# chlhnu/DOT-SOCP

Measured on AMD Instinct MI355X. Metric: ADMM iters/sec on NxNxT dot2d staggered grid at 1/2/4/8 MI355X, higher is better.
Workload: dtype f64

## Files before the change

### dot-socp_amd/capi.py

```python
import ctypes
import os

import numpy as np

_HERE = os.path.dirname(os.path.abspath(__file__))
LIB_PATH = os.path.join(_HERE, "lib", "libdotsocp.so")

i64 = ctypes.c_longlong
dbl = ctypes.c_double
vp = ctypes.c_void_p


class DotsocpError(RuntimeError):
    def __init__(self, code, msg):
        super().__init__(f"libdotsocp error {code}: {msg}")
        self.code = code


class Problem(ctypes.Structure):
    _fields_ = [("dim", ctypes.c_int), ("weighted", ctypes.c_int),
                ("ny", i64), ("nx", i64), ("nt", i64),
                ("D", dbl), ("E", dbl), ("cScale", dbl), ("dScale", dbl),
                ("normc", dbl), ("normd", dbl)]

# ... 16 lines not shown

METHOD_INPALM, METHOD_PALM, METHOD_ACCADMM = 0, 1, 2


F_PHI, F_Q, F_ALPHA, F_Z, F_BETA, F_C, F_WEIGHT = range(7)

SYMBOLS = {
    "dotsocp_last_error": (ctypes.c_char_p, []),
    "dotsocp_version": (ctypes.c_char_p, []),
    "dotsocp_device_count": (ctypes.c_int, []),
    "dotsocp_proj_soc": (ctypes.c_int, [vp, vp, i64, i64]),
    "dotsocp_bfd": (ctypes.c_int, [vp, vp, i64, i64, i64, dbl, dbl]),
    "dotsocp_bfd_conj": (ctypes.c_int, [vp, vp, i64, i64, i64, dbl]),
    "dotsocp_bfd1d": (ctypes.c_int, [vp, vp, i64, i64, dbl, dbl]),
    "dotsocp_bfd_conj1d": (ctypes.c_int, [vp, vp, i64, i64, dbl]),
    "dotsocp_oper_poisson": (ctypes.c_int, [vp, vp, i64, i64, i64, dbl]),
    "dotsocp_dctn": (ctypes.c_int, [vp, i64, i64, i64, ctypes.c_int]),
    "dotsocp_proj_soc_dev": (ctypes.c_int, [vp, vp, i64, i64, vp]),
    "dotsocp_bfd_dev": (ctypes.c_int, [vp, vp, i64, i64, i64, dbl, dbl, vp]),
    "dotsocp_bfd_conj_dev": (ctypes.c_int, [vp, vp, i64, i64, i64, dbl, vp]),
    "dotsocp_create": (vp, [ctypes.POINTER(Problem), ctypes.c_int, ctypes.c_int]),
    "dotsocp_create_multi": (vp, [ctypes.POINTER(Problem), ctypes.c_int, ctypes.c_int]),
    "dotsocp_destroy": (None, [vp]),
    "dotsocp_rccl_unique_id": (ctypes.c_int, [vp]),
    "dotsocp_attach_rccl": (ctypes.c_int, [vp, vp, ctypes.c_int, ctypes.c_int]),
    "dotsocp_slab_range": (ctypes.c_int, [i64, ctypes.c_int, ctypes.c_int, ctypes.POINTER(i64), ctypes.POINTER(i64)]),
    "dotsocp_field_len": (i64, [ctypes.POINTER(Problem), ctypes.c_int]),
    "dotsocp_dct_algorithm": (ctypes.c_int, [i64]),
    "dotsocp_dct_levels": (ctypes.c_int, [i64, ctypes.c_int]),
    "dotsocp_tsolve_tri_safe": (ctypes.c_int, [i64, i64, i64]),
    "dotsocp_cone_writes_beta": (ctypes.c_int, [i64, dbl, i64, ctypes.c_int, ctypes.c_int, ctypes.c_int, dbl, dbl]),
    "dotsocp_rescale_due": (ctypes.c_int, [i64, ctypes.c_int, dbl, dbl]),
    "dotsocp_qcone_form": (ctypes.c_int, [i64, dbl, i64, ctypes.c_int, ctypes.c_int, ctypes.c_int, ctypes.c_int, dbl, dbl]),
    "dotsocp_release_cache": (i64, []),
    "dotsocp_upload": (ctypes.c_int, [vp, ctypes.c_int, vp]),
    "dotsocp_upload_layers": (ctypes.c_int, [vp, ctypes.c_int, vp, i64, i64]),
    "dotsocp_download": (ctypes.c_int, [vp, ctypes.c_int, vp]),
    "dotsocp_begin": (ctypes.c_int, [vp, ctypes.POINTER(Opts)]),
    "dotsocp_begin_method": (ctypes.c_int, [vp, ctypes.POINTER(Opts), ctypes.c_int, ctypes.POINTER(AccOpts)]),
    "dotsocp_run": (ctypes.c_int, [vp, i64, ctypes.POINTER(i64)]),
    "dotsocp_recover_outputs": (ctypes.c_int, [vp, vp, vp, vp, vp, vp, vp, vp, vp]),
    "dotsocp_jump_next_level": (ctypes.c_int, [vp, vp]),
    "dotsocp_finish": (ctypes.c_int, [vp, ctypes.POINTER(Result)]),
    "dotsocp_get_history": (ctypes.c_int, [vp, vp, vp, vp, vp]),
    "dotsocp_set_profiling": (ctypes.c_int, [vp, ctypes.c_int]),
    "dotsocp_kernel_time": (ctypes.c_int, [vp, ctypes.c_char_p, ctypes.POINTER(dbl), ctypes.POINTER(i64)]),
    "dotsocp_canary_check": (ctypes.c_int, []),
    "dotsocp_poisson_phi": (ctypes.c_int, [vp]),
    "dotsocp_synchronize": (ctypes.c_int, [vp]),
    "dotsocp_weights_create": (vp, [ctypes.c_int, i64, i64, i64, ctypes.c_int]),
    "dotsocp_weights_destroy": (None, [vp]),
    "dotsocp_weights_len": (i64, [i64, i64, i64, ctypes.c_int, ctypes.c_int]),
    "dotsocp_weights_set": (ctypes.c_int, [vp, vp]),
    "dotsocp_weights_set_space": (ctypes.c_int, [vp, vp, vp]),
    "dotsocp_weights_restrict": (ctypes.c_int, [vp, ctypes.c_int]),
    "dotsocp_weights_log10_mean": (ctypes.c_int, [vp, ctypes.c_int, ctypes.POINTER(dbl)]),
    "dotsocp_weights_download": (ctypes.c_int, [vp, ctypes.c_int, vp]),
    "dotsocp_upload_weight_from": (ctypes.c_int, [vp, vp, ctypes.c_int]),
}

_lib = None


def _share_torchs_hip_runtime():
    import importlib.util
    import sys
# ... 68 lines not shown
```

### dot-socp_amd/csrc/capi.hip

```cpp
#include <cstring>
#include <new>

#include "comm.h"
#include "solver.h"
#include "weights.h"

using namespace dotsocp;

namespace dotsocp {
extern thread_local std::string g_last_error;
int dotsocp_slab_range_impl(i64 nt, int world, int rank, i64 *t0, i64 *t1);
}

struct dotsocp_ctx {
    Solver s;
};

struct dotsocp_weights {
    Weights w;
};

static int require_device() {
    int n = 0;
    if (hipGetDeviceCount(&n) != hipSuccess || n <= 0) {
// ... 243 lines not shown
    static_assert(sizeof(uid) == 128, "ncclUniqueId is expected to be 128 bytes");
    DS_NCCL(api.GetUniqueId(&uid));
    memcpy(id, &uid, sizeof uid);
    return 0;
}

int dotsocp_attach_rccl(dotsocp_ctx *ctx, const unsigned char id[128], int rank, int world) {
    if (!ctx) { set_error("ctx is NULL"); return DOTSOCP_EINVAL; }
    return ctx->s.attach_rccl(id, rank, world);
}

#define CTX_OR_FAIL()                                      \
    do {                                                   \
        if (!ctx) { set_error("ctx is NULL"); return DOTSOCP_EINVAL; } \
        (void)hipGetLastError();    \
    } while (0)

int dotsocp_dct_algorithm(dotsocp_i64 n) { return dct_choose_algorithm(n); }
int dotsocp_dct_levels(dotsocp_i64 n, int axis) { return dct_levels(n, axis); }
int dotsocp_tsolve_tri_safe(dotsocp_i64 ny, dotsocp_i64 nx, dotsocp_i64 nt) { return tsolve_tri_safe(ny, nx, nt) ? 1 : 0; }

int dotsocp_cone_writes_beta(dotsocp_i64 it, double last_sigma_it, dotsocp_i64 maxit, int check_step_by_step,
                             int last_of_run, int rescale, double maxFeas, double relGap) {
    return cone_writes_beta(it, last_sigma_it, maxit, check_step_by_step != 0, last_of_run != 0, rescale, maxFeas, relGap) ? 1 : 0;
}
int dotsocp_rescale_due(dotsocp_i64 it, int rescale, double maxFeas, double relGap) {
    return rescale_due(it, rescale, maxFeas, relGap) ? 1 : 0;
}
int dotsocp_qcone_form(dotsocp_i64 it, double last_sigma_it, dotsocp_i64 maxit, int check_step_by_step, int last_of_run,
                       int next_last_of_run, int rescale, double maxFeas, double relGap) {
    return qcone_form(it, last_sigma_it, maxit, check_step_by_step != 0, last_of_run != 0, next_last_of_run != 0, rescale,
                      maxFeas, relGap);
}

dotsocp_i64 dotsocp_field_len(const dotsocp_problem *p, int field) {
    if (!p || (p->dim != 1 && p->dim != 2) || p->nt < 2 || p->nx < 1 || (p->dim == 2 && p->ny < 1)) return -1;
    const i64 ny = p->dim == 1 ? p->nx : p->ny, nx = p->dim == 1 ? 1 : p->nx, nt = p->nt;
    const i64 Nphi = ny * nx * nt, Nz = ny * nx * (nt - 1);
    const i64 Nq = Nz + ny * (nx - 1) * nt + (ny - 1) * nx * nt;
    switch (field) {
        case DOTSOCP_F_PHI: case DOTSOCP_F_C: return Nphi;
        case DOTSOCP_F_Q: case DOTSOCP_F_ALPHA: case DOTSOCP_F_WEIGHT: return Nq;
        case DOTSOCP_F_Z: case DOTSOCP_F_BETA: return Nz * (p->dim == 1 ? 6 : 10);
        default: return -1;
    }
}

int dotsocp_upload(dotsocp_ctx *ctx, int field, const double *host) { CTX_OR_FAIL(); return ctx->s.upload(field, host); }
dotsocp_i64 dotsocp_release_cache(void) { return (dotsocp_i64)device_cache_release(); }

int dotsocp_upload_layers(dotsocp_ctx *ctx, int field, const double *host, dotsocp_i64 t0, dotsocp_i64 n) {
    CTX_OR_FAIL();
    return ctx->s.upload_layers(field, host, t0, n);
}
int dotsocp_download(dotsocp_ctx *ctx, int field, double *host) { CTX_OR_FAIL(); return ctx->s.download(field, host); }
int dotsocp_begin(dotsocp_ctx *ctx, const dotsocp_opts *opts) { CTX_OR_FAIL(); return ctx->s.begin(opts); }
int dotsocp_begin_method(dotsocp_ctx *ctx, const dotsocp_opts *opts, int method, const dotsocp_acc_opts *acc) {
    CTX_OR_FAIL();
    return ctx->s.begin_method(opts, method, acc);
}
int dotsocp_recover_outputs(dotsocp_ctx *ctx, const double *rho0, const double *rho1, double *rho, double *Ex,
                            double *Ey, double *q0, double *bx, double *by) {
    CTX_OR_FAIL();
    if (ctx->s.prob.dim == 1)
        return ctx->s.recover_outputs(rho0, rho1, rho, nullptr, Ex, q0, nullptr, bx);
    return ctx->s.recover_outputs(rho0, rho1, rho, Ex, Ey, q0, bx, by);
// ... 102 lines not shown
```

### dot-socp_amd/csrc/kernels.h

```cpp
#pragma once
#include "common.h"
#include "defer.h"

namespace dotsocp {

struct LoopCoef {
    double s;
    double sf;
    double dF;
    double at, ax, ay;
    double tau;
    double c1, c2;
    double dinv1, dinv2;
};

enum {
    S_Q2 = 0, S_Z2, S_APHI2, S_ALPHA2, S_BETA2, S_FBBETA2, S_PRIM1, S_PRIM2, S_DUAL1, S_DUAL2,
    S_COMPLEM, S_DOTCOMP, S_RHO2, S_RHOFQ2, S_MRHOB, S_M2, S_RHOB2, S_QALPHA, S_CPHI, S_PHI2,
    S_COUNT
};

struct KktCoef {
    double sigma;
    double kappa;
// ... 84 lines not shown

int launch_prolong_phi(const Grid &gf, const Grid &gc, const double *phic, double *phif, double sc_in, double sc_out,
                       hipStream_t st, i64 tc0 = 0);
int launch_prolong_beta(const Grid &gf, const Grid &gc, const double *betac, double *betaf, double *neg, double sc_in0,
                        double sc_in1, double sc_out, hipStream_t st, i64 tc0 = 0, i64 Nzc = -1);
int launch_scale_div(double *x, const double *w, i64 n, double sc, hipStream_t st);
int launch_fill(double *x, i64 n, double v, hipStream_t st);
int launch_outputs(const Grid &g, const double *q, const double *alpha, const double *weight, const double *rho0,
                   const double *rho1, const double *a_prev, double sig, double cD, double dD, int which, double *out,
                   hipStream_t st);
int launch_out_tail(const Grid &g, const double *alpha, const double *weight, double sig, double cD, double *out,
                    hipStream_t st);

struct QStepExtra {
    ScaleOps aops;
    double *partials, *resid;
    double kappa, dsD;
    double *u0_tail;
    int c_ends;
};
int launch_qstep_rhs(const Grid &g, const LoopCoef &c, const FusedGeom &fg, const double *phi, const double *q2,
                     const double *sx, const double *sy, const double *weight, const double *tail_bx,
                     const double *tail_by, const double *cvec, double *q_out, const double *alpha_in, double *alpha_out,
                     double *rhs, hipStream_t st, i64 z0 = 0, i64 zcount = -1, i64 zstride = 1,
                     const QStepExtra *ex = nullptr);
i64 qstep_rhs_blocks(const Grid &g, const FusedGeom &fg);
struct QConeArgs {
    const double *phi, *q2v, *sx, *sy, *cvec, *alpha_in, *gamma_in;
    double *alpha_out, *rhs, *q_out, *beta_out, *q2_out, *sx_out, *sy_out;
    i64 TC;
    int ap_on;
    double ap_mul, ap_div;
    int c_ends;
};
int launch_qcone(const Grid &g, const LoopCoef &c, const FusedGeom &fg, QConeArgs a, bool gout, hipStream_t st);
i64 qcone_chunk_len(const Grid &g);
i64 qstep_rhs_chunks(const Grid &g, const FusedGeom &fg, i64 *TC = nullptr);
int launch_qstep_rhs_acc(int var, const Grid &g, const LoopCoef &c, const FusedGeom &fg, const double *phi,
                         const double *q2, const double *sx, const double *sy, const double *weight, const double *cvec,
                         double *q_raw, const double *alpha_in, double *alpha_out, double *rhs, double *q_state,
                         const double *q_anchor, const double *alpha_anchor, const AccCoef &k, hipStream_t st,
                         const double *tail_bx = nullptr, const double *tail_by = nullptr, double *u0_tail = nullptr);
int launch_qstep_palm_first(const Grid &g, const LoopCoef &c, const FusedGeom &fg, const double *phi, const double *q2,
                            const double *sx, const double *sy, const double *cvec, double *q_out, const double *alpha,
                            double *rhs, hipStream_t st, const double *tail_bx = nullptr, const double *tail_by = nullptr,
                            const double *qk = nullptr);

int launch_qstep_fused(const Grid &g, const LoopCoef &c, const FusedGeom &fg, const double *phi,
                       const double *q2, const double *sx, const double *sy, const double *weight,
                       const double *tail_bx, const double *tail_by, double *q_out, double *alpha,
                       hipStream_t st);
int launch_rhs_sigma_fix(const Grid &g, double *rhs, const double *r, double *cvec, double factor, hipStream_t st,
                         bool c_ends = false);
int launch_c_interior_test(const Grid &g, const double *cvec, int *flag, hipStream_t st);
int launch_rhs_fixup(const Grid &g, const LoopCoef &c, const double *u0_prev, double *rhs, hipStream_t st);
int launch_grad(const Grid &g, const LoopCoef &c, const double *phi, double *out, hipStream_t st);
int launch_tail_finalize(const Grid &g, const LoopCoef &c, const FusedGeom &fg, const double *q2, const double *sx,
                         const double *sy, double *tail_bx, double *tail_by, hipStream_t st);
int launch_kkt_tail(const Grid &g, const double *alpha, const double *beta, const double *weight, double *a0,
                    double *a0w, double *bt_bx, double *bt_by, hipStream_t st);
int launch_rhs(const Grid &g, const LoopCoef &c, const double *q, const double *alpha, const double *cvec,
               const double *weight, const double *u0_prev, double *rhs, hipStream_t st, bool c_ends = false);
int launch_qstep(const Grid &g, const LoopCoef &c, const double *phi, const double *z, const double *beta,
                 const double *weight, const double *tail_bx, const double *tail_by, double *q,
                 double *alpha, hipStream_t st);
int launch_u0_tail(const Grid &g, const double *q, const double *alpha, const double *weight, double *out,
                   hipStream_t st);
int launch_scale(double *x, i64 n, double mul, double div, hipStream_t st);
// ... 79 lines not shown
```

### dot-socp_amd/csrc/qstep_march.hip

```cpp
#include "device_utils.h"
#include "gather_tile.h"
#include "kernels.h"
#include "qstep_tile.h"

#include <cstdlib>

namespace dotsocp {


struct QRhsArgs {
    const double *phi, *q2v, *sx, *sy, *weight, *tail_bx, *tail_by, *cvec, *alpha_in;
    double *q_out, *alpha_out, *rhs;
    double *u0_tail;
    i64 TC, z0, zstride;
    double *q_state;
    const double *q_anchor, *alpha_anchor;
    double c1, c2, om_rho, rho;
    APend ap;
    int xcd;
    const double *qk;
    double *partials, *resid;
    double kappa, dsD;
    int c_ends;
};
// ... 234 lines not shown
    if (z0 < 0 || zcount <= 0 || zstride < 1 || z0 + (zcount - 1) * zstride >= chunks) return 0;
    a.TC = TC;
    a.z0 = z0;
    a.zstride = zstride;
    a.xcd = 1;
    dim3 grid((unsigned)fg.nyblk, (unsigned)fg.nxblk, (unsigned)zcount);
    dim3 blk(TILE_Y, TILE_X);
    const char *qe = getenv("DOTSOCP_QTX");
    const int qtx_env = qe ? atoi(qe) : 0;
    const int qtx = qtx_env ? qtx_env : ((fg.nyblk * fg.nxblk * zcount >= 8192 && !a.weight) ? 2 * TILE_X : TILE_X);
    if (var == 0 && !a.partials && qtx == 2 * TILE_X) {
        dim3 grid2((unsigned)fg.nyblk, (unsigned)((g.nx + 2 * TILE_X - 1) / (2 * TILE_X)), (unsigned)zcount);
        dim3 blk2(TILE_Y, 2 * TILE_X);
        if (a.weight) DS_KLAUNCH((k_qstep_rhs<true, 0, false, 2 * TILE_X>), grid2, blk2, 0, st, g, c, fg, a);
        else DS_KLAUNCH((k_qstep_rhs<false, 0, false, 2 * TILE_X>), grid2, blk2, 0, st, g, c, fg, a);
        DS_HIP(hipGetLastError());
        return 0;
    }
#define QRHS_LAUNCH(W, V) DS_KLAUNCH((k_qstep_rhs<W, V>), grid, blk, 0, st, g, c, fg, a)
    if (var == 0 && a.partials) {
        if (a.weight) DS_KLAUNCH((k_qstep_rhs<true, 0, true>), grid, blk, 0, st, g, c, fg, a);
        else DS_KLAUNCH((k_qstep_rhs<false, 0, true>), grid, blk, 0, st, g, c, fg, a);
    } else if (a.weight) {
        if (var == 0) QRHS_LAUNCH(true, 0); else if (var == 1) QRHS_LAUNCH(true, 1); else QRHS_LAUNCH(true, 2);
    } else {
        if (var == 0) QRHS_LAUNCH(false, 0); else if (var == 1) QRHS_LAUNCH(false, 1);
        else if (var == 2) QRHS_LAUNCH(false, 2); else QRHS_LAUNCH(false, 3);
    }
#undef QRHS_LAUNCH
    DS_HIP(hipGetLastError());
    return 0;
}

template <bool NT, bool GOUT>
__global__ void __launch_bounds__(TILE_Y *TILE_X, 3) k_qcone(Grid g, LoopCoef c, FusedGeom fg, QConeArgs a) {
    constexpr int XB = TILE_X;
    __shared__ double2 xch[2][XB][TILE_Y];
    __shared__ double ph[2][XB + 2][TILE_Y + 2];
    __shared__ double2 gch[2][XB][64];
    const APend ap{a.ap_on, a.ap_mul, a.ap_div};
    const BlockId blk = block_id(true);
    const QTile<XB> t = q_tile<XB>(g, fg, blk);
    const int lane = t.lane, xl = t.xl;
    const i64 y = t.y, x = t.x;
    const bool inb = t.inb;
    const i64 t0 = (i64)blk.z * a.TC;
    const i64 t1 = (t0 + a.TC < g.ntl) ? t0 + a.TC : g.ntl;
    const i64 tstart = (t0 >= 2) ? t0 - 2 : 0;
    const i64 tstop = (t1 == g.ntl) ? t1 + 1 : t1;
    const i64 nxblk = gridDim.y, nyblk = gridDim.x;
    const QSrc src{a.phi, a.q2v, a.sx, a.sy, nullptr, nullptr, nullptr, a.cvec, a.alpha_in, nullptr, a.c_ends};
    double p0 = 0.0;
    if (inb) {
        const i64 node0 = y + g.py * (x + g.nx * tstart);
        p0 = a.phi[node0];
        store_phi_layer<XB>(ph[0], t, p0, load_phi_halo(g, t, a.phi, node0));
    }
    double u0prev = 0.0;
    double q0c = 0.0;
    EdgeQuad eprev{0.0, 0.0, 0.0, 0.0};
    GatherCarry gc;
    int par = 0;
    __syncthreads();
    for (i64 tl = tstart; tl < tstop; ++tl) {
        const bool own = tl >= t0;
        const bool hasC = (tl > tstart) && (tl - 1 < g.ncl);
        const i64 ci = t.yc + g.py * (t.xc + g.nx * (hasC ? tl - 1 : 0));
        double b[10];
        if (hasC) {
#pragma unroll
            for (int j = 0; j < 10; ++j) b[j] = ld_stream<NT>(a.gamma_in + j * g.Nc + ci);
        }
        EdgeQuad ecur{0.0, 0.0, 0.0, 0.0};
        double q0n = 0.0;
        if (tl < g.ntl) {
            const QLayerIn in = q_layer_load<false, XB>(g, c, fg, t, src, ph[par], tl, false, false);
            const QLayerOut o = q_layer_calc<false, 0, XB>(c, t, in, ap, p0, false, false);
            q0n = o.q0n;
            if (own) {
                if (in.hasCell) {
                    a.alpha_out[in.node] = o.a0n;
                    if (!GOUT) a.q_out[in.node] = o.q0n;
                }
                if (t.hasBx) {
                    a.alpha_out[in.eX] = o.aXn;
                    if (!GOUT) a.q_out[in.eX] = o.qXn;
                }
                if (t.hasBy) {
                    a.alpha_out[in.eY] = o.aYn;
                    if (!GOUT) a.q_out[in.eY] = o.qYn;
                }
            }
            xch[par][xl][lane] = make_double2(o.ubx, o.qXn);
            store_phi_layer<XB>(ph[par ^ 1], t, in.pTl, in.h);
            __syncthreads();
            const double uby_s = __shfl_up(o.uby, 1, 64);
            const double qY_s = __shfl_up(o.qYn, 1, 64);
            if (inb) {
                const double2 r = from_left(t, xch[par], make_double2(o.ubx_l, o.qL),
                                            make_double2(0.0, 0.0));
                const double uby_m = from_below(t, uby_s, o.uby_b), qY_m = from_below(t, qY_s, o.qB);
                if (own) a.rhs[in.node] = adjoint_sum(g, c, t, tl, u0prev, o.u0, r.x, o.ubx, uby_m, o.uby) + in.cv;
                ecur.xm = (x >= 1) ? c.sf * r.y : 0.0;
                ecur.xp = (x <= g.nx - 2) ? c.sf * o.qXn : 0.0;
                ecur.ym = (y >= 1) ? c.sf * qY_m : 0.0;
                ecur.yp = (y <= g.ny - 2) ? c.sf * o.qYn : 0.0;
            }
            u0prev = o.u0;
            p0 = o.pT;
            par ^= 1;
        }
        if (tl > tstart) {
            double w[10];
            if (hasC) {
                double v[10];
                build_z2(v, q0c, eprev, ecur, c.s, c.dF);
#pragma unroll
                for (int j = 0; j < 10; ++j) b[j] = mult_finish(b[j], v[j], c.tau);
                if (!GOUT && own && inb) {
#pragma unroll
                    for (int j = 0; j < 10; ++j) st_stream<NT>(a.beta_out + j * g.Nc + ci, b[j]);
                }
#pragma unroll
                for (int j = 0; j < 10; ++j) v[j] = v[j] - b[j];
                proj_row<10>(v);
                if (GOUT && own && inb) {
#pragma unroll
                    for (int j = 0; j < 10; ++j) st_stream<NT>(a.beta_out + j * g.Nc + ci, mult_carry(b[j], v[j], c.tau));
                }
#pragma unroll
                for (int j = 0; j < 10; ++j) w[j] = v[j] + b[j];
                if (own && inb) a.q2_out[ci] = c.s * (w[9] - w[0]);
            } else {
#pragma unroll
                for (int j = 0; j < 10; ++j) w[j] = 0.0;
            }
            gather_emit<XB>(g, c.sf, gch, gc, w, tl - 1, own && inb, x, y, xl, lane, nxblk, nyblk, blk.y, blk.x, a.q2_out,
                            a.sx_out, a.sy_out);
        }
        eprev = ecur;
        q0c = q0n;
    }
}

i64 qcone_chunk_len(const Grid &g) {
    i64 TC = g.ntl;
    if (const char *e = getenv("DOTSOCP_QCONE_TC")) {
        const i64 n = atoll(e);
        if (n >= 1) TC = n;
    }
    return TC < g.ntl ? TC : g.ntl;
}

int launch_qcone(const Grid &g, const LoopCoef &c, const FusedGeom &fg, QConeArgs a, bool gout, hipStream_t st) {
    if (fg.XB != TILE_X || !(g.first && g.last) || g.ncl < 1) { set_error("internal: k_qcone on a grid it does not serve"); return DOTSOCP_ESTATE; }
    a.TC = qcone_chunk_len(g);
    const i64 chunks = (g.ntl + a.TC - 1) / a.TC;
    dim3 grid((unsigned)fg.nyblk, (unsigned)fg.nxblk, (unsigned)chunks);
    dim3 blk(TILE_Y, TILE_X);
    const bool nt = stream_nt_enabled();
    if (gout) {
        if (nt) DS_KLAUNCH((k_qcone<true, true>), grid, blk, 0, st, g, c, fg, a);
        else DS_KLAUNCH((k_qcone<false, true>), grid, blk, 0, st, g, c, fg, a);
    } else {
        if (nt) DS_KLAUNCH((k_qcone<true, false>), grid, blk, 0, st, g, c, fg, a);
        else DS_KLAUNCH((k_qcone<false, false>), grid, blk, 0, st, g, c, fg, a);
    }
    DS_HIP(hipGetLastError());
    return 0;
}

int launch_qstep_palm_first(const Grid &g, const LoopCoef &c, const FusedGeom &fg, const double *phi, const double *q2,
                            const double *sx, const double *sy, const double *cvec, double *q_out, const double *alpha,
                            double *rhs, hipStream_t st, const double *tail_bx, const double *tail_by, const double *qk) {
    QRhsArgs a{};
    a.phi = phi; a.q2v = q2; a.sx = sx; a.sy = sy; a.cvec = cvec; a.tail_bx = tail_bx; a.tail_by = tail_by;
    a.alpha_in = alpha; a.q_out = q_out; a.rhs = rhs; a.qk = qk;
    return launch_qstep_rhs_var(3, g, c, fg, a, st);
}

}
```

### dot-socp_amd/csrc/solver.h

```cpp
#pragma once
#include <chrono>
#include <functional>
#include <memory>
#include <string>
#include <vector>

#include "hostmem.h"
#include "kernels.h"

namespace dotsocp {

int guarded_malloc(void **p, size_t bytes);
void guarded_free(void *p);
long long device_cache_release();
int canary_check(std::string *report);
bool canary_enabled();
bool stream_stress_enabled();
void stream_stress(hipStream_t st);

template <class T>
inline int dmalloc(T **p, i64 n) {
    *p = nullptr;
    if (n <= 0) n = 1;
    return guarded_malloc((void **)p, sizeof(T) * (size_t)n);
// ... 47 lines not shown
    double *u0_prev = nullptr, *tail_bx = nullptr, *tail_by = nullptr;
    double *a0_prev = nullptr, *a0w_prev = nullptr, *btail_bx = nullptr, *btail_by = nullptr;
    double *send_plane = nullptr, *send_plane2 = nullptr, *send_bx = nullptr, *send_by = nullptr;
    KktWork kw{};
    double *q_old = nullptr, *q2 = nullptr, *beta2 = nullptr, *sx = nullptr, *sy = nullptr;
    double *q3 = nullptr, *p2 = nullptr, *sxp = nullptr, *syp = nullptr;
    double *send_pbx = nullptr, *send_pby = nullptr, *ptail_bx = nullptr, *ptail_by = nullptr;
    double *alpha2 = nullptr;
    double *sx2 = nullptr, *sy2 = nullptr;
    double *tri_send = nullptr, *tri_recv = nullptr, *tri_bsend = nullptr, *tri_brecv = nullptr, *tri_zero = nullptr;
    double *carry = nullptr;
    FusedGeom fg{};
    double *phi_p = nullptr, *alpha_p = nullptr, *z_p = nullptr;
    double *phi_a = nullptr, *q_a = nullptr, *alpha_a = nullptr, *z_a = nullptr, *beta_a = nullptr;
};

#define FOR_SLABS(s) for (auto &s : slabs) if (int rc_use__ = use(s)) return rc_use__; else

int dotsocp_slab_range_impl(i64 nt, int world, int rank, i64 *t0, i64 *t1);
void pencil_range(i64 plane, int world, int j, i64 *l0, i64 *l1);

bool if_adjust_sigma(double iter, double last_iter);

enum Phase { PH_RHS = 0, PH_POISSON, PH_PROJ, PH_QSTEP, PH_BETA, PH_KKT, PH_FUSED_A, PH_FUSED_B, PH_MATERIALISE,
             PH_COMM, PH_INTERP, PH_ACC_CONE, PH_ACC_GATHER, PH_QSTEP0, PH_TRANSPOSE, PH_CONE_CARRY, PH_QCONE, PH_COUNT };

bool rescale_due(i64 it, int rescale, double maxFeas, double relGap);
bool cone_writes_beta(i64 it, double lastSigmaIt, i64 maxit, bool checkStepByStep, bool last_of_run, int rescale,
                      double maxFeas, double relGap);

enum { QCONE_NONE = 0, QCONE_STEADY = 1, QCONE_EXIT = 2 };
int qcone_form(i64 it, double lastSigmaIt, i64 maxit, bool checkStepByStep, bool last_of_run, bool next_last_of_run,
               int rescale, double maxFeas, double relGap);

struct Solver {
    dotsocp_problem prob{};
    int device = 0;
    i64 ny = 0, nx = 0, nt = 0;
    hipStream_t stream = nullptr;
    hipStream_t stream_z = nullptr;
    bool multi_device = false;
    int ndev_visible = 1;
    std::vector<DevRes *> devres;
    int cur_dev = -1;
    std::vector<Slab> slabs;
    std::unique_ptr<DeferCtx> defer;
    int world = 1;
    int rank = 0;
    void *nccl = nullptr;
    double *h_sums = nullptr;
    double *d_red = nullptr;
    bool fused = true;
    bool overlap = false;
    bool tri_tsolve = true;
    bool peer_ok = true;
    bool cross_device = false;
    ~Solver();
    int init(const dotsocp_problem *p, int device, int nslabs, bool multi_dev = false);
    int attach_rccl(const unsigned char *id, int rank, int world);
    int use(const Slab &s);
    int use_dev(int d);
    int sync_all();
    DevRes *res_for(int dev);
    i64 column_pad() const;
    i64 row_pitch() const;
    int alloc_slabs(int first, int count);
// ... 52 lines not shown
    int upload_weight_from(const double *src, int src_dev, i64 src_ny, i64 src_nx, i64 src_nt);
    bool c_ends_on = true;
    int detect_c_ends();
    int recover_outputs(const double *rho0, const double *rho1, double *rho, double *Ex, double *Ey, double *q0,
                        double *bx, double *by);
    int jump_from(Solver &coarse);

    bool begun = false, finished = false, stopped = false;
    dotsocp_opts opts{};
    bool checkPrimDualFeas = true;
    double time_limit = 3600.0;
    double sigma = 1.0, sigmaScale = 1.0;
    double cScale = 1.0, dScale = 1.0, D = 1.0, E = 1.0;
    double norm_c = 0.0, norm_d = 0.0;
    double h = 1.0;
    int rescale = 0, use_feasOrg = 0;
    double maxFeas = 0.0, relGap = 0.0, tol_feasOrg = 0.0;
    double lastSigmaIt = 0.0;
    i64 it = 0;
    LoopCoef lc{};
    std::vector<double> hist_kkt, hist_time, hist_iter, hist_gap;
    std::chrono::steady_clock::time_point t_begin;
    double elapsed_prev = 0.0;
    double elapsed_agreed = 0.0;
    bool deferred = false;
    bool z_valid = true;
    bool z_prev_ok = false;
    bool rhs_valid = false;
    bool cone_carry = true;
    bool beta_gamma = false;
    bool cone_gout = false;
    bool last_of_run = false;
    int qcone = -1;
    bool q_valid = true;
    bool early_pass = false;
    bool early_gout = false;
    bool next_last_of_run = false;
    int need_q(const char *who) const;
    int qcone_decide() const;
    bool time_limit_passed() const;
    i64 timeout_at = -1;
    bool timeout_pending = false;
    int need_beta_form(const char *who) const;
    ScaleOps bops{0, 1.0, 1.0, 1.0, 1.0};
    ScaleOps zp_ops{0, 1.0, 1.0, 1.0, 1.0};
    int push_beta_op(double mul, double div);
    int flush_beta();
    ScaleOps aops{0, 1.0, 1.0, 1.0, 1.0};
    int flush_alpha();
    int sigma_scale_folded(double factor);
    FusedArgs pending_step_args(const Slab &s) const;
    double last_S[S_COUNT] = {0};
    double last_S_sigma = 1.0;
    i64 last_S_it = -1;
    bool norm_cache = true;
    bool kkt_fold = true;
    KktCoef kkt_coef() const;
    int clear_partials(Slab &s);
    int begin(const dotsocp_opts *o);
    int begin_method(const dotsocp_opts *o, int method, const dotsocp_acc_opts *acc);
    int run(i64 n_iters, i64 *done);
    int finish(dotsocp_result *res);
    int step(bool *brk);
    int rescale_block();
    int poisson_all(const PhiHooks *hooks = nullptr);
    int poisson_phi();
// ... 48 lines not shown
```

### dot-socp_amd/csrc/solver.hip

```cpp
#include "solver.h"

#include <algorithm>
#include <cmath>
#include <cstring>

#include "comm.h"

namespace dotsocp {

void Solver::update_coef() {
    lc.s = E / D;
    lc.sf = edge_factor(lc.s);
    lc.dF = E / dScale;
    const double ht = 1.0 / (double)(nt - 1);
    lc.at = D * (1.0 / ht);
    lc.ax = (nx > 1) ? D * (1.0 / (1.0 / (double)(nx - 1))) : 0.0;
    lc.ay = (ny > 1) ? D * (1.0 / (1.0 / (double)(ny - 1))) : 0.0;
    lc.tau = opts.tau;
    const double tmp = (E / D) * (E / D);
    if (prob.weighted) { lc.c1 = 2.0 * tmp; lc.c2 = tmp; }
    else { lc.c1 = 1.0 + 2.0 * tmp; lc.c2 = 1.0 + tmp; }
    lc.dinv1 = 1.0 / lc.c1;
    lc.dinv2 = 1.0 / lc.c2;
}
// ... 94 lines not shown
    if (m == DOTSOCP_METHOD_INPALM) return begin(o);
    DS_ARG(m == DOTSOCP_METHOD_ACCADMM || m == DOTSOCP_METHOD_PALM, "unknown method");
    DS_ARG(prob.dim == 2, "the reference has PALM and acc-ADMM loops for 2-D problems only");
    DS_ARG(!(m == DOTSOCP_METHOD_PALM && prob.weighted), "the reference has no weighted PALM loop");
    method = m;
    int rc = begin(o);
    if (rc != 0) { method = DOTSOCP_METHOD_INPALM; return rc; }
    return (m == DOTSOCP_METHOD_PALM) ? palm_begin() : acc_begin(acc);
}

int Solver::begin(const dotsocp_opts *o) {
    DS_ARG(o != nullptr, "opts is NULL");
    DS_ARG(o->maxit >= 0, "opts.maxit < 0");
    DS_ARG(o->sigma > 0, "opts.sigma must be positive");
    if (begun) { set_error("begin() called twice"); return DOTSOCP_ESTATE; }
    cur_dev = -1;
    DS_CHECK(use_dev(device));
    DS_CHECK(ensure_alloc());
    if (method == DOTSOCP_METHOD_ACCADMM) {
        DS_CHECK(acc_alloc());
        fused = false;
    }
    opts = *o;
    cone_carry = true;
    if (const char *e = getenv("DOTSOCP_CONE_CARRY")) cone_carry = (atoi(e) != 0);
    c_ends_on = true;
    if (const char *e = getenv("DOTSOCP_C_ENDS")) c_ends_on = (atoi(e) != 0);
    if (c_ends_on) DS_CHECK(detect_c_ends());
    timeout_at = -1;
    if (const char *e = getenv("DOTSOCP_TEST_TIMEOUT_AT")) timeout_at = atoll(e);
    qcone = -1;
    if (const char *e = getenv("DOTSOCP_QCONE")) qcone = atoi(e);
    if (qcone < -1 || qcone > 2) qcone = -1;
    q_valid = true;
    early_pass = false;
    early_gout = false;
    next_last_of_run = false;
    beta_gamma = false;
    cone_gout = false;
    last_of_run = false;
    timeout_pending = false;
    checkPrimDualFeas = (o->checkPrimDualFeas < 0) ? !prob.weighted : (o->checkPrimDualFeas != 0);
    time_limit = (o->time_limit > 0) ? o->time_limit : 3600.0;
    sigma = o->sigma;
    lastSigmaIt = -INFINITY;
    cScale = prob.cScale; dScale = prob.dScale; D = prob.D; E = prob.E;
    use_feasOrg = 0;
    tol_feasOrg = 5 * o->tol;
    rescale = o->scaling ? 1 : 0;
    maxFeas = INFINITY; relGap = INFINITY;
    h = 1.0 / ((double)nx * (double)ny * (double)nt);
    norm_c = prob.normc; norm_d = prob.normd;
    update_coef();
    DS_CHECK(scale_state(1.0, sigma, 1.0, true));
    DS_CHECK(exchange_q_halo(false));
    sigmaScale = 1.0;
    it = 0;
    stopped = false;
    deferred = false;
    z_valid = true;
    z_prev_ok = false;
    rhs_valid = false;
    last_S_it = -1;
    hist_kkt.clear(); hist_time.clear(); hist_iter.clear(); hist_gap.clear();
    for (int i = 0; i < PH_COUNT; ++i) { phase_ms[i] = 0; phase_launches[i] = 0; }
    if (canary_enabled() && getenv("DOTSOCP_CANARY_SELFTEST")) {
// ... 142 lines not shown
        }
        const int mode = deferred ? 1 : 0;
        if (s.carry && C > 1) {
            for (i64 z = z0; z < z0 + zc; ++z) {
                a.carry_in = (z > 0) ? s.carry : nullptr;
                a.carry_out = (z + 1 < C) ? s.carry : nullptr;
                DS_CHECK(launch_cone_fused(mode, s.g, lc, s.fg, a, s.st, z, 1, flavour));
            }
        } else {
            DS_CHECK(launch_cone_fused(mode, s.g, lc, s.fg, a, s.st, z0, zc, flavour));
        }
        if (deferred && part != 1) std::swap(s.beta, s.beta2);
    }
    prof_end(ph);
    if (part == 1) return 0;
    if (deferred) {
        bops.clear();
        beta_gamma = gout;
    }
    return 0;
}

KktCoef Solver::kkt_coef() const {
    KktCoef k;
    k.sigma = sigma;
    k.kappa = sigma * cScale * D;
    k.dsD = dScale / D;
    k.dsE = dScale / E;
    return k;
}

int Solver::phase_q(int part, bool kkt, int early) {
    if (!fused) DS_CHECK(flush_alpha());
    if (early != QCONE_NONE && (part != 0 || kkt || multi() || !fused || !deferred || !beta_gamma || !bops.empty())) {
        set_error("internal: early cone pass in a state it does not serve");
        return DOTSOCP_ESTATE;
    }
    const bool egout = (early == QCONE_STEADY);
    const int ph = (early != QCONE_NONE) ? PH_QCONE : PH_QSTEP;
    prof_begin(ph);
    FOR_SLABS(s) {
        hipStream_t st = s.st;
        if (early != QCONE_NONE && qcone != 2) {
            if (!s.sx2) {
                DS_CHECK(s.zalloc(&s.sx2, s.fg.sx_len));
                DS_CHECK(s.zalloc(&s.sy2, s.fg.sy_len));
            }
            QConeArgs a{};
            a.phi = s.phi; a.q2v = s.q2; a.sx = s.sx; a.sy = s.sy; a.cvec = s.c; a.alpha_in = s.alpha; a.gamma_in = s.beta;
            a.alpha_out = s.alpha2; a.rhs = s.w0; a.q_out = s.q_old; a.beta_out = s.beta2;
            a.q2_out = s.q; a.sx_out = s.sx2; a.sy_out = s.sy2;
            a.ap_on = aops.n; a.ap_mul = aops.mul; a.ap_div = aops.div;
            a.c_ends = (c_ends_on && s.c_ends) ? 1 : 0;
            DS_CHECK(launch_qcone(s.g, lc, s.fg, a, egout, st));
            std::swap(s.alpha, s.alpha2);
            std::swap(s.q, s.q_old);
            std::swap(s.q2, s.q_old);
            std::swap(s.sx, s.sx2);
            std::swap(s.sy, s.sy2);
            std::swap(s.beta, s.beta2);
        } else if (!fused) {
            DS_CHECK(launch_qstep(s.g, lc, s.phi, s.z, s.beta, s.weight, s.tail_bx, s.tail_by, s.q, s.alpha, s.st));
        } else {
            const i64 C = qstep_rhs_chunks(s.g, s.fg);
            i64 z0 = 0, zc = C, zs = 1;
            if (part == 1) { zc = C - 1; }
            else if (part == 2) { z0 = C - 1; zc = 1; }
            QStepExtra ex{};
            ex.aops = aops;
            ex.c_ends = (c_ends_on && s.c_ends) ? 1 : 0;
            if (multi() && !s.g.last && part != 1) ex.u0_tail = s.send_plane;
            if (kkt) {
                const KktCoef k = kkt_coef();
                ex.partials = kkt_qstep_partials(s.g, s.kw);
                ex.resid = s.w1;
                ex.kappa = k.kappa; ex.dsD = k.dsD;
            }
            DS_CHECK(launch_qstep_rhs(s.g, lc, s.fg, s.phi, s.q2, s.sx, s.sy, s.weight, s.tail_bx, s.tail_by, s.c,
                                      s.q_old, s.alpha, s.alpha2, s.w0, st, z0, zc, zs, &ex));
            if (part != 1) std::swap(s.alpha, s.alpha2);
            if (part != 1) std::swap(s.q, s.q_old);
            if (early != QCONE_NONE) {
                FusedArgs a{};
                a.q = s.q; a.q2 = s.q2; a.sx = s.sx; a.sy = s.sy;
                a.beta_in = s.beta; a.beta_out = s.beta2;
                a.bops = bops;
                DS_CHECK(launch_cone_fused(1, s.g, lc, s.fg, a, s.st, 0, s.fg.chunks, CONE_GIN | (egout ? CONE_GOUT : 0)));
                std::swap(s.beta, s.beta2);
            }
        }
    }
    prof_end(ph);
    if (part == 1) return 0;
    q_valid = true;
    if (early != QCONE_NONE) {
        q_valid = !egout || qcone == 2;
        beta_gamma = egout;
        z_valid = false;
        z_prev_ok = false;
        early_pass = true;
        early_gout = egout;
    }
    u0_made = multi() && fused;
    if (fused) aops.clear();
    rhs_valid = fused;
    if (multi() && fused && comm_z && cone_split_enabled()) halo_pending = true;
    else DS_CHECK(exchange_q_halo(true));
    return 0;
}

int Solver::phase_mult() {
    if (fused) {
        deferred = true;
        return 0;
    }
    prof_begin(PH_BETA);
    FOR_SLABS(s) DS_CHECK(launch_beta_update(s.g, lc, s.q, s.z, s.beta, s.st));
    prof_end(PH_BETA);
    return 0;
}

int Solver::materialise() {
    if (!fused || !deferred) return 0;
    DS_CHECK(need_beta_form("materialise"));
    DS_CHECK(need_q("materialise"));
    DS_CHECK(ensure_halo());
    prof_begin(PH_MATERIALISE);
    FOR_SLABS(s) {
        FusedArgs a = pending_step_args(s);
        a.beta_out = s.beta;
        a.z_out = s.z;
        DS_CHECK(launch_cone_fused(2, s.g, lc, s.fg, a, s.st));
    }
    prof_end(PH_MATERIALISE);
// ... 172 lines not shown
    DS_CHECK(scale_state(dScale2, cScale2 * cScale2, dScale2, true));
    if (method == DOTSOCP_METHOD_PALM) {
        FOR_SLABS(s) DS_CHECK(launch_scale(s.phi, s.g.NphiAlloc, 1.0, dScale2, s.st));
    }
    dScale = dScale2 * dScale;
    cScale = cScale2 * cScale;
    sigmaScale = sigmaScale * (cScale2 / dScale2);
    update_coef();
    rescale += 1;
    return 0;
}

bool rescale_due(i64 it, int rescale, double maxFeas, double relGap) {
    if (rescale >= 3 && (it % 100) == 0) return true;
    if (rescale == 1 && maxFeas < 2e-2 && it >= 10 && relGap < 5e-2) return true;
    if (rescale == 2 && maxFeas < 5e-3 && it >= 50 && relGap < 1e-2) return true;
    return false;
}

bool cone_writes_beta(i64 it, double lastSigmaIt, i64 maxit, bool checkStepByStep, bool last_of_run, int rescale,
                      double maxFeas, double relGap) {
    if (checkStepByStep || if_adjust_sigma((double)it, lastSigmaIt) || it >= maxit) return true;
    if (last_of_run) return true;
    return rescale_due(it + 1, rescale, maxFeas, relGap);
}

int qcone_form(i64 it, double lastSigmaIt, i64 maxit, bool checkStepByStep, bool last_of_run, bool next_last_of_run,
               int rescale, double maxFeas, double relGap) {
    if (cone_writes_beta(it, lastSigmaIt, maxit, checkStepByStep, last_of_run, rescale, maxFeas, relGap)) return QCONE_NONE;
    return cone_writes_beta(it + 1, lastSigmaIt, maxit, checkStepByStep, next_last_of_run, rescale, maxFeas, relGap)
               ? QCONE_EXIT : QCONE_STEADY;
}

bool Solver::time_limit_passed() const {
    return timeout_pending || (remote() ? false : (elapsed() > time_limit || (timeout_at > 0 && it >= timeout_at)));
}

int Solver::qcone_decide() const {
    if (qcone == 0 || !fused || multi() || prob.weighted || method != DOTSOCP_METHOD_INPALM) return QCONE_NONE;
    if (!deferred || !beta_gamma || !bops.empty()) return QCONE_NONE;
    const Slab &s = slabs[0];
    if (s.g.ncl < 1 || s.fg.XB != 4) return QCONE_NONE;
    if (qcone < 0 && s.fg.nyblk * s.fg.nxblk < 2048) return QCONE_NONE;
    if (time_limit_passed()) return QCONE_NONE;
    return qcone_form(it, lastSigmaIt, opts.maxit, opts.ifCheckStepByStep != 0, last_of_run, next_last_of_run, rescale,
                      maxFeas, relGap);
}

bool if_adjust_sigma(double iter, double last_iter) {
    const double passed = iter - last_iter;
    if (iter < 20 && passed >= 3) return true;
    if (iter < 50 && passed >= 6) return true;
    if (iter < 100 && passed >= 10) return true;
    if (iter < 200 && passed >= 15) return true;
    if (iter < 500 && passed >= 25) return true;
    return passed >= 40;
}

static const double kUpdateRule[11][2] = {
    {1.1, 1.10}, {1.2, 1.15}, {1.5, 1.20}, {2, 1.26}, {2.5, 1.28}, {3.33, 1.32},
    {5, 1.35}, {10, 1.40}, {20, 1.60}, {40, 1.80}, {50, 2.00}};

static double get_factor(double xi) {
    double factor = 1.0;
    for (int i = 0; i < 11; ++i) {
        if (xi >= kUpdateRule[i][0]) factor = kUpdateRule[i][1];
        else break;
    }
    return factor;
}

static void adjust_lagrangian_param(double &sigma, double xi, double &factor) {
    factor = 1.0;
    if (xi >= 1) factor = get_factor(xi);
    else if (xi < 1) factor = 1.0 / get_factor(1.0 / xi);
    if (factor != 1.0) {
        const double old = sigma;
// ... 275 lines not shown
```

### include/dotsocp.h

```cpp
#ifndef DOTSOCP_H
#define DOTSOCP_H

#ifdef __cplusplus
extern "C" {
#endif

typedef long long dotsocp_i64;

enum {
    DOTSOCP_OK = 0,
    DOTSOCP_EINVAL = -1,
    DOTSOCP_ENODEVICE = -2,
    DOTSOCP_EHIP = -3,
    DOTSOCP_ESTATE = -4,
    DOTSOCP_ECOMM = -5
};

const char *dotsocp_last_error(void);
const char *dotsocp_version(void);
int dotsocp_device_count(void);
dotsocp_i64 dotsocp_release_cache(void);


int dotsocp_proj_soc(double *out, const double *in, dotsocp_i64 M, dotsocp_i64 K);
// ... 67 lines not shown
typedef struct {
    double sigma;
    double sigma_internal;
    double cScale, dScale;
    double times[7];
    dotsocp_i64 iters;
    dotsocp_i64 hist_len;
    int stopped;
    double time_extra;
} dotsocp_result;

dotsocp_ctx *dotsocp_create(const dotsocp_problem *prob, int device, int nslabs);
dotsocp_ctx *dotsocp_create_multi(const dotsocp_problem *prob, int first_device, int ngpu);
void dotsocp_destroy(dotsocp_ctx *ctx);

int dotsocp_rccl_unique_id(unsigned char id[128]);
int dotsocp_attach_rccl(dotsocp_ctx *ctx, const unsigned char id[128], int rank, int world);

int dotsocp_slab_range(dotsocp_i64 nt, int world, int rank, dotsocp_i64 *t0, dotsocp_i64 *t1);

dotsocp_i64 dotsocp_field_len(const dotsocp_problem *prob, int field);

int dotsocp_dct_algorithm(dotsocp_i64 n);

int dotsocp_dct_levels(dotsocp_i64 n, int axis);

int dotsocp_tsolve_tri_safe(dotsocp_i64 ny, dotsocp_i64 nx, dotsocp_i64 nt);

int dotsocp_cone_writes_beta(dotsocp_i64 it, double last_sigma_it, dotsocp_i64 maxit, int check_step_by_step,
                             int last_of_run, int rescale, double maxFeas, double relGap);
int dotsocp_rescale_due(dotsocp_i64 it, int rescale, double maxFeas, double relGap);
int dotsocp_qcone_form(dotsocp_i64 it, double last_sigma_it, dotsocp_i64 maxit, int check_step_by_step, int last_of_run,
                       int next_last_of_run, int rescale, double maxFeas, double relGap);

int dotsocp_upload(dotsocp_ctx *ctx, int field, const double *host);
int dotsocp_download(dotsocp_ctx *ctx, int field, double *host);
int dotsocp_upload_layers(dotsocp_ctx *ctx, int field, const double *host, dotsocp_i64 t0, dotsocp_i64 n);

int dotsocp_begin(dotsocp_ctx *ctx, const dotsocp_opts *opts);
int dotsocp_begin_method(dotsocp_ctx *ctx, const dotsocp_opts *opts, int method, const dotsocp_acc_opts *acc);
int dotsocp_run(dotsocp_ctx *ctx, dotsocp_i64 n_iters, dotsocp_i64 *done);
int dotsocp_finish(dotsocp_ctx *ctx, dotsocp_result *res);

int dotsocp_recover_outputs(dotsocp_ctx *ctx, const double *rho0, const double *rho1, double *rho, double *Ex,
                            double *Ey, double *q0, double *bx, double *by);

int dotsocp_jump_next_level(dotsocp_ctx *coarse, dotsocp_ctx *fine);

typedef struct dotsocp_weights dotsocp_weights;

dotsocp_weights *dotsocp_weights_create(int device, dotsocp_i64 ny, dotsocp_i64 nx, dotsocp_i64 nt, int levels);
void dotsocp_weights_destroy(dotsocp_weights *w);

dotsocp_i64 dotsocp_weights_len(dotsocp_i64 ny, dotsocp_i64 nx, dotsocp_i64 nt, int levels, int level);

int dotsocp_weights_set(dotsocp_weights *w, const double *weight);
int dotsocp_weights_set_space(dotsocp_weights *w, const double *weightX, const double *weightY);

int dotsocp_weights_restrict(dotsocp_weights *w, int log_mean);

int dotsocp_weights_log10_mean(dotsocp_weights *w, int level, double *mean);

int dotsocp_weights_download(dotsocp_weights *w, int level, double *host);

int dotsocp_upload_weight_from(dotsocp_ctx *ctx, dotsocp_weights *w, int level);

// ... 16 lines not shown
```

Measured before the change: 98.10.

## Add entry form of fused q-cone pass consuming beta without gamma

```diff
diff --git a/dot-socp_amd/capi.py b/dot-socp_amd/capi.py
--- a/dot-socp_amd/capi.py
+++ b/dot-socp_amd/capi.py
@@ -72,6 +72,8 @@
     "dotsocp_cone_writes_beta": (ctypes.c_int, [i64, dbl, i64, ctypes.c_int, ctypes.c_int, ctypes.c_int, dbl, dbl]),
     "dotsocp_rescale_due": (ctypes.c_int, [i64, ctypes.c_int, dbl, dbl]),
     "dotsocp_qcone_form": (ctypes.c_int, [i64, dbl, i64, ctypes.c_int, ctypes.c_int, ctypes.c_int, ctypes.c_int, dbl, dbl]),
+    "dotsocp_qcone_entry_form": (ctypes.c_int, [i64, dbl, i64, ctypes.c_int, ctypes.c_int, ctypes.c_int, ctypes.c_int, dbl, dbl,
+                                                ctypes.c_int]),
     "dotsocp_release_cache": (i64, []),
     "dotsocp_upload": (ctypes.c_int, [vp, ctypes.c_int, vp]),
     "dotsocp_upload_layers": (ctypes.c_int, [vp, ctypes.c_int, vp, i64, i64]),
diff --git a/dot-socp_amd/csrc/capi.hip b/dot-socp_amd/csrc/capi.hip
--- a/dot-socp_amd/csrc/capi.hip
+++ b/dot-socp_amd/csrc/capi.hip
@@ -299,6 +299,11 @@
     return qcone_form(it, last_sigma_it, maxit, check_step_by_step != 0, last_of_run != 0, next_last_of_run != 0, rescale,
                       maxFeas, relGap);
 }
+int dotsocp_qcone_entry_form(dotsocp_i64 it, double last_sigma_it, dotsocp_i64 maxit, int check_step_by_step, int last_of_run,
+                             int next_last_of_run, int rescale, double maxFeas, double relGap, int pass_left_gamma) {
+    return qcone_entry_form(it, last_sigma_it, maxit, check_step_by_step != 0, last_of_run != 0, next_last_of_run != 0, rescale,
+                            maxFeas, relGap, pass_left_gamma != 0) ? 1 : 0;
+}
 
 dotsocp_i64 dotsocp_field_len(const dotsocp_problem *p, int field) {
     if (!p || (p->dim != 1 && p->dim != 2) || p->nt < 2 || p->nx < 1 || (p->dim == 2 && p->ny < 1)) return -1;
diff --git a/dot-socp_amd/csrc/kernels.h b/dot-socp_amd/csrc/kernels.h
--- a/dot-socp_amd/csrc/kernels.h
+++ b/dot-socp_amd/csrc/kernels.h
@@ -140,8 +140,10 @@
     int ap_on;
     double ap_mul, ap_div;
     int c_ends;
-};
-int launch_qcone(const Grid &g, const LoopCoef &c, const FusedGeom &fg, QConeArgs a, bool gout, hipStream_t st);
+    const double *qk;
+    ScaleOps bops;
+};
+int launch_qcone(const Grid &g, const LoopCoef &c, const FusedGeom &fg, QConeArgs a, bool gout, hipStream_t st, bool gin = true);
 i64 qcone_chunk_len(const Grid &g);
 i64 qstep_rhs_chunks(const Grid &g, const FusedGeom &fg, i64 *TC = nullptr);
 int launch_qstep_rhs_acc(int var, const Grid &g, const LoopCoef &c, const FusedGeom &fg, const double *phi,
diff --git a/dot-socp_amd/csrc/qstep_march.hip b/dot-socp_amd/csrc/qstep_march.hip
--- a/dot-socp_amd/csrc/qstep_march.hip
+++ b/dot-socp_amd/csrc/qstep_march.hip
@@ -290,8 +290,9 @@
     return 0;
 }
 
-template <bool NT, bool GOUT>
-__global__ void __launch_bounds__(TILE_Y *TILE_X, 3) k_qcone(Grid g, LoopCoef c, FusedGeom fg, QConeArgs a) {
+template <bool NT, bool GIN, bool GOUT>
+__global__ void __launch_bounds__(TILE_Y *TILE_X, GIN ? 3 : 2) k_qcone(Grid g, LoopCoef c, FusedGeom fg, QConeArgs a) {
+    static_assert(GIN || GOUT, "the beta-in, beta-out pass stays a kernel of its own");
     constexpr int XB = TILE_X;
     __shared__ double2 xch[2][XB][TILE_Y];
     __shared__ double ph[2][XB + 2][TILE_Y + 2];
@@ -317,6 +318,7 @@
     double u0prev = 0.0;
     double q0c = 0.0;
     EdgeQuad eprev{0.0, 0.0, 0.0, 0.0};
+    EdgeQuad eoprev{0.0, 0.0, 0.0, 0.0};
     GatherCarry gc;
     int par = 0;
     __syncthreads();
@@ -328,6 +330,12 @@
         if (hasC) {
 #pragma unroll
             for (int j = 0; j < 10; ++j) b[j] = ld_stream<NT>(a.gamma_in + j * g.Nc + ci);
+        }
+        EdgeQuad eocur{0.0, 0.0, 0.0, 0.0};
+        double q0o = 0.0;
+        if constexpr (!GIN) {
+            eocur = load_edges(g, a.qk, t.yc, t.xc, (tl < g.ntl) ? tl : g.ntl - 1, c.sf);
+            q0o = a.qk[ci];
         }
         EdgeQuad ecur{0.0, 0.0, 0.0, 0.0};
         double q0n = 0.0;
@@ -372,12 +380,23 @@
             double w[10];
             if (hasC) {
                 double v[10];
+                if constexpr (!GIN) apply_scale_ops(b, a.bops);
                 build_z2(v, q0c, eprev, ecur, c.s, c.dF);
-#pragma unroll
-                for (int j = 0; j < 10; ++j) b[j] = mult_finish(b[j], v[j], c.tau);
-                if (!GOUT && own && inb) {
-#pragma unroll
-                    for (int j = 0; j < 10; ++j) st_stream<NT>(a.beta_out + j * g.Nc + ci, b[j]);
+                if constexpr (GIN) {
+#pragma unroll
+                    for (int j = 0; j < 10; ++j) b[j] = mult_finish(b[j], v[j], c.tau);
+                    if (!GOUT && own && inb) {
+#pragma unroll
+                        for (int j = 0; j < 10; ++j) st_stream<NT>(a.beta_out + j * g.Nc + ci, b[j]);
+                    }
+                } else {
+                    double zo[10];
+                    build_z2(zo, q0o, eoprev, eocur, c.s, c.dF);
+#pragma unroll
+                    for (int j = 0; j < 10; ++j) zo[j] = zo[j] - b[j];
+                    proj_row<10>(zo);
+#pragma unroll
+                    for (int j = 0; j < 10; ++j) b[j] = mult_finish(mult_carry(b[j], zo[j], c.tau), v[j], c.tau);
                 }
 #pragma unroll
                 for (int j = 0; j < 10; ++j) v[j] = v[j] - b[j];
@@ -397,6 +416,7 @@
                             a.sx_out, a.sy_out);
         }
         eprev = ecur;
+        if constexpr (!GIN) eoprev = eocur;
         q0c = q0n;
     }
 }
@@ -410,19 +430,24 @@
     return TC < g.ntl ? TC : g.ntl;
 }
 
-int launch_qcone(const Grid &g, const LoopCoef &c, const FusedGeom &fg, QConeArgs a, bool gout, hipStream_t st) {
+int launch_qcone(const Grid &g, const LoopCoef &c, const FusedGeom &fg, QConeArgs a, bool gout, hipStream_t st, bool gin) {
     if (fg.XB != TILE_X || !(g.first && g.last) || g.ncl < 1) { set_error("internal: k_qcone on a grid it does not serve"); return DOTSOCP_ESTATE; }
+    if (!gin && (!gout || !a.qk || a.qk == a.q2_out || a.qk == a.q_out)) { set_error("internal: k_qcone's entry form with bad arguments"); return DOTSOCP_ESTATE; }
+    if (gin && !a.bops.empty()) { set_error("internal: gamma with a pending scaling"); return DOTSOCP_ESTATE; }
     a.TC = qcone_chunk_len(g);
     const i64 chunks = (g.ntl + a.TC - 1) / a.TC;
     dim3 grid((unsigned)fg.nyblk, (unsigned)fg.nxblk, (unsigned)chunks);
     dim3 blk(TILE_Y, TILE_X);
     const bool nt = stream_nt_enabled();
-    if (gout) {
-        if (nt) DS_KLAUNCH((k_qcone<true, true>), grid, blk, 0, st, g, c, fg, a);
-        else DS_KLAUNCH((k_qcone<false, true>), grid, blk, 0, st, g, c, fg, a);
+    if (!gin) {
+        if (nt) DS_KLAUNCH((k_qcone<true, false, true>), grid, blk, 0, st, g, c, fg, a);
+        else DS_KLAUNCH((k_qcone<false, false, true>), grid, blk, 0, st, g, c, fg, a);
+    } else if (gout) {
+        if (nt) DS_KLAUNCH((k_qcone<true, true, true>), grid, blk, 0, st, g, c, fg, a);
+        else DS_KLAUNCH((k_qcone<false, true, true>), grid, blk, 0, st, g, c, fg, a);
     } else {
-        if (nt) DS_KLAUNCH((k_qcone<true, false>), grid, blk, 0, st, g, c, fg, a);
-        else DS_KLAUNCH((k_qcone<false, false>), grid, blk, 0, st, g, c, fg, a);
+        if (nt) DS_KLAUNCH((k_qcone<true, true, false>), grid, blk, 0, st, g, c, fg, a);
+        else DS_KLAUNCH((k_qcone<false, true, false>), grid, blk, 0, st, g, c, fg, a);
     }
     DS_HIP(hipGetLastError());
     return 0;
diff --git a/dot-socp_amd/csrc/solver.h b/dot-socp_amd/csrc/solver.h
--- a/dot-socp_amd/csrc/solver.h
+++ b/dot-socp_amd/csrc/solver.h
@@ -103,6 +103,9 @@
 enum { QCONE_NONE = 0, QCONE_STEADY = 1, QCONE_EXIT = 2 };
 int qcone_form(i64 it, double lastSigmaIt, i64 maxit, bool checkStepByStep, bool last_of_run, bool next_last_of_run,
                int rescale, double maxFeas, double relGap);
+enum { QCONE_ENTRY = 3 };
+bool qcone_entry_form(i64 it, double lastSigmaIt, i64 maxit, bool checkStepByStep, bool last_of_run, bool next_last_of_run,
+                      int rescale, double maxFeas, double relGap, bool pass_left_gamma);
 
 struct Solver {
     dotsocp_problem prob{};
@@ -221,6 +224,7 @@
     bool cone_gout = false;
     bool last_of_run = false;
     int qcone = -1;
+    int qcone_entry = 1;
     bool q_valid = true;
     bool early_pass = false;
     bool early_gout = false;
diff --git a/dot-socp_amd/csrc/solver.hip b/dot-socp_amd/csrc/solver.hip
--- a/dot-socp_amd/csrc/solver.hip
+++ b/dot-socp_amd/csrc/solver.hip
@@ -150,6 +150,8 @@
     qcone = -1;
     if (const char *e = getenv("DOTSOCP_QCONE")) qcone = atoi(e);
     if (qcone < -1 || qcone > 2) qcone = -1;
+    qcone_entry = 1;
+    if (const char *e = getenv("DOTSOCP_QCONE_ENTRY")) qcone_entry = (atoi(e) != 0);
     q_valid = true;
     early_pass = false;
     early_gout = false;
@@ -358,16 +360,36 @@
 
 int Solver::phase_q(int part, bool kkt, int early) {
     if (!fused) DS_CHECK(flush_alpha());
-    if (early != QCONE_NONE && (part != 0 || kkt || multi() || !fused || !deferred || !beta_gamma || !bops.empty())) {
+    const bool entry = (early == QCONE_ENTRY);
+    if (early != QCONE_NONE && (part != 0 || kkt || multi() || !fused ||
+                                (entry ? (beta_gamma || !q_valid) : (!deferred || !beta_gamma || !bops.empty())))) {
         set_error("internal: early cone pass in a state it does not serve");
         return DOTSOCP_ESTATE;
     }
-    const bool egout = (early == QCONE_STEADY);
+    const bool egout = (early == QCONE_STEADY) || entry;
     const int ph = (early != QCONE_NONE) ? PH_QCONE : PH_QSTEP;
     prof_begin(ph);
     FOR_SLABS(s) {
         hipStream_t st = s.st;
-        if (early != QCONE_NONE && qcone != 2) {
+        if (entry && qcone != 2) {
+            if (!s.sx2) {
+                DS_CHECK(s.zalloc(&s.sx2, s.fg.sx_len));
+                DS_CHECK(s.zalloc(&s.sy2, s.fg.sy_len));
+            }
+            QConeArgs a{};
+            a.phi = s.phi; a.q2v = s.q2; a.sx = s.sx; a.sy = s.sy; a.cvec = s.c; a.alpha_in = s.alpha; a.gamma_in = s.beta;
+            a.qk = s.q; a.bops = bops;
+            a.alpha_out = s.alpha2; a.rhs = s.w0; a.q_out = nullptr; a.beta_out = s.beta2;
+            a.q2_out = s.q_old; a.sx_out = s.sx2; a.sy_out = s.sy2;
+            a.ap_on = aops.n; a.ap_mul = aops.mul; a.ap_div = aops.div;
+            a.c_ends = (c_ends_on && s.c_ends) ? 1 : 0;
+            DS_CHECK(launch_qcone(s.g, lc, s.fg, a, true, st, false));
+            std::swap(s.alpha, s.alpha2);
+            std::swap(s.q2, s.q_old);
+            std::swap(s.sx, s.sx2);
+            std::swap(s.sy, s.sy2);
+            std::swap(s.beta, s.beta2);
+        } else if (early != QCONE_NONE && qcone != 2) {
             if (!s.sx2) {
                 DS_CHECK(s.zalloc(&s.sx2, s.fg.sx_len));
                 DS_CHECK(s.zalloc(&s.sy2, s.fg.sy_len));
@@ -411,7 +433,8 @@
                 a.q = s.q; a.q2 = s.q2; a.sx = s.sx; a.sy = s.sy;
                 a.beta_in = s.beta; a.beta_out = s.beta2;
                 a.bops = bops;
-                DS_CHECK(launch_cone_fused(1, s.g, lc, s.fg, a, s.st, 0, s.fg.chunks, CONE_GIN | (egout ? CONE_GOUT : 0)));
+                if (entry) a.q_old = s.q_old;
+                DS_CHECK(launch_cone_fused(1, s.g, lc, s.fg, a, s.st, 0, s.fg.chunks, (entry ? 0 : CONE_GIN) | (egout ? CONE_GOUT : 0)));
                 std::swap(s.beta, s.beta2);
             }
         }
@@ -426,6 +449,7 @@
         z_prev_ok = false;
         early_pass = true;
         early_gout = egout;
+        if (entry) bops.clear();
     }
     u0_made = multi() && fused;
     if (fused) aops.clear();
@@ -664,17 +688,29 @@
                ? QCONE_EXIT : QCONE_STEADY;
 }
 
+bool qcone_entry_form(i64 it, double lastSigmaIt, i64 maxit, bool checkStepByStep, bool last_of_run, bool next_last_of_run,
+                      int rescale, double maxFeas, double relGap, bool pass_left_gamma) {
+    if (pass_left_gamma) return false;
+    return qcone_form(it, lastSigmaIt, maxit, checkStepByStep, last_of_run, next_last_of_run, rescale, maxFeas, relGap) ==
+           QCONE_STEADY;
+}
+
 bool Solver::time_limit_passed() const {
     return timeout_pending || (remote() ? false : (elapsed() > time_limit || (timeout_at > 0 && it >= timeout_at)));
 }
 
 int Solver::qcone_decide() const {
     if (qcone == 0 || !fused || multi() || prob.weighted || method != DOTSOCP_METHOD_INPALM) return QCONE_NONE;
-    if (!deferred || !beta_gamma || !bops.empty()) return QCONE_NONE;
     const Slab &s = slabs[0];
     if (s.g.ncl < 1 || s.fg.XB != 4) return QCONE_NONE;
     if (qcone < 0 && s.fg.nyblk * s.fg.nxblk < 2048) return QCONE_NONE;
     if (time_limit_passed()) return QCONE_NONE;
+    if (!beta_gamma) {
+        if (!qcone_entry || !cone_carry || !q_valid) return QCONE_NONE;
+        return qcone_entry_form(it, lastSigmaIt, opts.maxit, opts.ifCheckStepByStep != 0, last_of_run, next_last_of_run, rescale,
+                                maxFeas, relGap, false) ? QCONE_ENTRY : QCONE_NONE;
+    }
+    if (!deferred || !bops.empty()) return QCONE_NONE;
     return qcone_form(it, lastSigmaIt, opts.maxit, opts.ifCheckStepByStep != 0, last_of_run, next_last_of_run, rescale,
                       maxFeas, relGap);
 }
diff --git a/include/dotsocp.h b/include/dotsocp.h
--- a/include/dotsocp.h
+++ b/include/dotsocp.h
@@ -123,6 +123,8 @@
 int dotsocp_rescale_due(dotsocp_i64 it, int rescale, double maxFeas, double relGap);
 int dotsocp_qcone_form(dotsocp_i64 it, double last_sigma_it, dotsocp_i64 maxit, int check_step_by_step, int last_of_run,
                        int next_last_of_run, int rescale, double maxFeas, double relGap);
+int dotsocp_qcone_entry_form(dotsocp_i64 it, double last_sigma_it, dotsocp_i64 maxit, int check_step_by_step, int last_of_run,
+                             int next_last_of_run, int rescale, double maxFeas, double relGap, int pass_left_gamma);
 
 int dotsocp_upload(dotsocp_ctx *ctx, int field, const double *host);
 int dotsocp_download(dotsocp_ctx *ctx, int field, double *host);
```

After: 99.31 (median of 6 runs). 1.2% higher.
